# xl-tang3/RCOT

Measured on AMD Instinct MI355X. Metric: 128x128 patches/sec (gen+critic step), higher is better.
Workload: dtype fp32 (exact fp32 MFMA everywhere); 1 GPU; BASELINE configs[1]: Restormer T_net(decoder=True)+F_net(128), denoise_50, RMSprop, paired, B=8/GPU 128x128; global_batch=8, patch=128, parallelism=dp1, gemm_prec=fp32

## Files before the change

### include/rcot_hip.h

```cpp
#ifndef RCOT_HIP_H
#define RCOT_HIP_H
#include <stddef.h>

#ifdef __cplusplus
extern "C" {
#endif

#define RCOT_ABI_VERSION 41

#define RCOT_PREC_FP32 0
#define RCOT_PREC_BF16X3 1
#define RCOT_PREC_BF16X6 2
#define RCOT_PREC_BF16X1 3

int rcot_abi_version(void);
int rcot_debug_nt_coop(int mask);
int rcot_profile_begin(void);
int rcot_profile_end(char* out, int n);
int rcot_last_kernel(char* out, int n);

int rcot_conv1x1_fwd(const float* W, long ldw, const float* X, long sXb, float* Y, long sYb, int B, int Ci, int Co,
                     int N, const float* ln_mu, const float* ln_rs, const float* ln_w, const float* ln_b,
                     const float* R, long sRb, float beta, void* stream);
int rcot_conv1x1_dgrad(const float* W, long ldw, const float* dY, long sdYb, float* dX, long sdXb, int B, int Ci,
                       int Co, int N, float beta, void* stream);
int rcot_conv1x1_wgrad(const float* dY, long sdYb, const float* X, long sXb, float* dW, long ldw, int B, int Ci,
                       int Co, int N, const float* ln_mu, const float* ln_rs, const float* ln_w, const float* ln_b,
                       float beta, float* ws, size_t ws_bytes, int prec, void* stream);
int rcot_conv1x1_wgrad_slabs(const float* dY, long sdYb, const float* X, long sXb, int B, int Ci, int Co, int N,
                             const float* ln_mu, const float* ln_rs, const float* ln_w, const float* ln_b, float* ws,
                             size_t ws_bytes, int prec, int* S, int* ldws, void* stream);
int rcot_conv1x1_dgrad_wgrad_slabs(const float* WP, long ldp, const void* WPs, const float* dY, long sdYb, float* dX, long sdXb,
                                   const float* X, long sXb, int B, int Ci, int Co, int N, const float* ln_mu,
                                   const float* ln_rs, const float* ln_w, const float* ln_b, float* ws, size_t ws_bytes,
                                   float* ws_slabs, size_t ws_slabs_bytes, int prec, int* S, int* ldws, void* stream);

int rcot_bmm_nn(const float* A, long lda, long sAo, long sAi, int transA, const float* Bm, long ldb, long sBo,
                long sBi, float* C, long ldc, long sCo, long sCi, const float* R, long ldr, long sRo, long sRi,
                const float* rowscale, long sSo, long sSi, int Zo, int Zi, int M, int N, int K, float beta,
                void* stream);
int rcot_bmm_nt(const float* A, long lda, long sAo, long sAi, const float* Bm, long ldb, long sBo, long sBi,
                float* C, long ldc, long sCo, long sCi, int Zo, int Zi, int M, int N, int K, float* ws,
                size_t ws_bytes, int prec, void* stream);

int rcot_bmm_nt_slabs(const float* A, long lda, long sAo, long sAi, const float* Bm, long ldb, long sBo, long sBi, int Zo, int Zi,
                      int M, int N, int K, float* ws, size_t ws_bytes, int prec, int* S, int* ldws, void* stream);

int rcot_gemm_kmajor(const float* At, long lda, long sAo, long sAi, int a_rows, const float* Bm, long ldb, long sBo,
                     long sBi, float* C, long ldc, long sCo, long sCi, const float* R, long ldr, long sRo, long sRi,
                     const float* rowscale, long sSo, long sSi, float* ln_mu, float* ln_rs, long sLN, int ln_compute,
                     const float* ln_w, const float* ln_b, const float* AtF, const float* ln_c12, const void* Asplit, int Zo,
                     int Zi, int M, int N, int K, float beta, float* ws, size_t ws_bytes, int prec, void* stream);
typedef struct rcot_kmajor_desc {
    const float* At; long lda, sAo, sAi; int a_rows;
// ... 194 lines not shown
```

### rcot_amd/csrc/pointwise.hip

```cpp
#include <cstdlib>
#include "common.h"
#include "../../include/rcot_hip.h"

using namespace rcot;

namespace {

constexpr int LN_TX = 16, LN_TY = 16, LN_PIX = LN_TX * 4;

__device__ __forceinline__ float4 f4_add(float4 a, float4 b) { return make_float4(a.x + b.x, a.y + b.y, a.z + b.z, a.w + b.w); }

template <int TX>
__device__ __forceinline__ float4 reduce_rows(float4 v, float4* red, int tx, int ty) {
    constexpr int TY = 256 / TX;
    __syncthreads();
    red[ty * TX + tx] = v;
    __syncthreads();
    float4 t = red[tx];
#pragma unroll
    for (int i = 1; i < TY; ++i) t = f4_add(t, red[i * TX + tx]);
    return t;
}

__global__ __launch_bounds__(256) void ln_stats_kernel(const float* __restrict__ x, float* __restrict__ mu,
// ... 159 lines not shown
        if (r < rows) s0 += p[(long)r * C2];
    }
    red[rl][cl] = s0 + s1;
    __syncthreads();
    if (rl == 0 && col < C2) {
        float s = 0.f;
#pragma unroll
        for (int i = 0; i < 32; ++i) s += red[i][cl];
        if (col < C) dw[col] += s;
        else db[col - C] += s;
    }
}

struct SlabSets {
    const float* ws[4];
    float* dst[4];
    int S[4], M[4], N[4], ldws[4];
    int per[4];
    long ldd[4];
    int chunk0[5];
    int n;
};

__global__ __launch_bounds__(1024) void block_param_reduce_kernel(const float* __restrict__ part1, const float* __restrict__ part2,
                                                                  int rows, int C, float* __restrict__ gw1, float* __restrict__ gb1,
                                                                  float* __restrict__ gw2, float* __restrict__ gb2,
                                                                  const float* __restrict__ dWo_part, float* __restrict__ gWo,
                                                                  const float* __restrict__ dtemp_part, float* __restrict__ gtemp,
                                                                  int B, int heads, int nw, SlabSets ss) {
    __shared__ float red[32][33];
    const int nl = (2 * C + 31) / 32;
    const int blk = blockIdx.x;
    if (blk >= 2 * nl + nw) {
        const int cb = blk - 2 * nl - nw;
        int d = 0;
        while (d + 1 < ss.n && cb >= ss.chunk0[d + 1]) ++d;
        const int c = cb - ss.chunk0[d];
        const long mn = (long)ss.M[d] * ss.N[d];
        const long slab = (long)ss.M[d] * ss.ldws[d];
        if (ss.S[d] <= 8) {
            const unsigned Nn = (unsigned)ss.N[d], mnu = (unsigned)mn, S = (unsigned)ss.S[d];
            const unsigned ldw = (unsigned)ss.ldws[d];
            const float* wsb = ss.ws[d];
            float* dstb = ss.dst[d];
            float v[4][8], old[4];
            long doff[4];
            bool ok[4];
#pragma unroll
            for (int j = 0; j < 4; ++j) {
                const unsigned idx = (unsigned)c * 4096u + 1024u * j + threadIdx.x;
                ok[j] = idx < mnu;
                const unsigned ic = ok[j] ? idx : mnu - 1;
                const unsigned m = ic / Nn, n = ic - m * Nn;
                const float* w = wsb + (size_t)m * ldw + n;
                doff[j] = (long)m * ss.ldd[d] + n;
#pragma unroll
                for (unsigned u = 0; u < 8; ++u) {
                    const unsigned uc = u < S ? u : S - 1;
                    v[j][u] = w[(long)uc * slab];
                }
                old[j] = dstb[doff[j]];
            }
#pragma unroll
            for (int j = 0; j < 4; ++j) {
#pragma unroll
                for (unsigned u = 0; u < 8; ++u) v[j][u] = u < S ? v[j][u] : 0.f;
                const float sum = ((v[j][0] + v[j][1]) + (v[j][2] + v[j][3])) + ((v[j][4] + v[j][5]) + (v[j][6] + v[j][7]));
                if (ok[j]) dstb[doff[j]] = old[j] + sum;
            }
            return;
        }
        if (ss.per[d] == 256) {
            const int o = threadIdx.x & 255, q = threadIdx.x >> 8;
            const long idx = (long)c * 256 + o;
            float* part = &red[0][0];
            float a = 0.f;
            int m = 0, n = 0;
            if (idx < mn) {
                m = (int)(idx / ss.N[d]);
                n = (int)(idx - (long)m * ss.N[d]);
                const float* w = ss.ws[d] + (long)m * ss.ldws[d] + n;
                float acc8[8];
#pragma unroll
                for (int u = 0; u < 8; ++u) acc8[u] = 0.f;
                int s = q;
                for (; s + 28 < ss.S[d]; s += 32) {
#pragma unroll
                    for (int u = 0; u < 8; ++u) acc8[u] += w[(long)(s + 4 * u) * slab];
                }
                for (; s < ss.S[d]; s += 4) acc8[0] += w[(long)s * slab];
                a = ((acc8[0] + acc8[1]) + (acc8[2] + acc8[3])) + ((acc8[4] + acc8[5]) + (acc8[6] + acc8[7]));
            }
            part[q * 256 + o] = a;
            __syncthreads();
            if (q == 0 && idx < mn)
                ss.dst[d][(long)m * ss.ldd[d] + n] += (part[o] + part[256 + o]) + (part[512 + o] + part[768 + o]);
            return;
        }
        const int o = threadIdx.x & 255, q = threadIdx.x >> 8;
        const unsigned Nn = (unsigned)ss.N[d], mnu = (unsigned)mn, ldw = (unsigned)ss.ldws[d];
        const int S = ss.S[d];
        float a[4];
        long doff[4];
        bool ok[4];
        const float* w[4];
#pragma unroll
        for (int j = 0; j < 4; ++j) {
            const unsigned idx = (unsigned)c * 1024u + 256u * j + o;
            ok[j] = idx < mnu;
            const unsigned ic = ok[j] ? idx : mnu - 1;
            const unsigned m = ic / Nn, n = ic - m * Nn;
            w[j] = ss.ws[d] + (size_t)m * ldw + n;
            doff[j] = (long)m * ss.ldd[d] + n;
        }
        float acc8[4][8];
#pragma unroll
        for (int j = 0; j < 4; ++j)
#pragma unroll
            for (int u = 0; u < 8; ++u) acc8[j][u] = 0.f;
        int sl = q;
        for (; sl + 28 < S; sl += 32) {
#pragma unroll
            for (int j = 0; j < 4; ++j)
#pragma unroll
                for (int u = 0; u < 8; ++u) acc8[j][u] += w[j][(long)(sl + 4 * u) * slab];
        }
        for (; sl < S; sl += 4) {
#pragma unroll
            for (int j = 0; j < 4; ++j) acc8[j][0] += w[j][(long)sl * slab];
        }
#pragma unroll
        for (int j = 0; j < 4; ++j)
            a[j] = ((acc8[j][0] + acc8[j][1]) + (acc8[j][2] + acc8[j][3])) + ((acc8[j][4] + acc8[j][5]) + (acc8[j][6] + acc8[j][7]));
        __shared__ float part4[4][1024];
#pragma unroll
        for (int j = 0; j < 4; ++j) part4[q][256 * j + o] = a[j];
        __syncthreads();
        {
            const int t = threadIdx.x;
            const unsigned idx = (unsigned)c * 1024u + t;
            if (idx < mnu) {
                const unsigned m = idx / Nn, n = idx - m * Nn;
                ss.dst[d][(long)m * ss.ldd[d] + n] += (part4[0][t] + part4[1][t]) + (part4[2][t] + part4[3][t]);
            }
        }
        (void)doff; (void)ok;
        return;
    }
    if (blk < 2 * nl) {
        const float* part = blk < nl ? part1 : part2;
        float* dw = blk < nl ? gw1 : gw2;
        float* db = blk < nl ? gb1 : gb2;
        const int cb = blk < nl ? blk : blk - nl;
        const int cl = threadIdx.x & 31, rl = threadIdx.x >> 5;
        const int col = cb * 32 + cl, C2 = 2 * C;
        float a8[8];
#pragma unroll
        for (int u = 0; u < 8; ++u) a8[u] = 0.f;
        if (col < C2) {
            const float* p = part + col;
            int r = rl;
            for (; r + 224 < rows; r += 256) {
#pragma unroll
                for (int u = 0; u < 8; ++u) a8[u] += p[(long)(r + 32 * u) * C2];
            }
            for (; r < rows; r += 32) a8[0] += p[(long)r * C2];
        }
        red[rl][cl] = ((a8[0] + a8[1]) + (a8[2] + a8[3])) + ((a8[4] + a8[5]) + (a8[6] + a8[7]));
        __syncthreads();
// ... 5 lines not shown
            else db[col - C] += s;
        }
        return;
    }
    const long n = (long)C * C;
    const long i = (long)(blk - 2 * nl) * 1024 + threadIdx.x;
    if (i < n) {
        float s = 0.f;
        int b = 0;
        for (; b + 8 <= B; b += 8) {
            float v[8];
#pragma unroll
            for (int u = 0; u < 8; ++u) v[u] = dWo_part[(long)(b + u) * n + i];
#pragma unroll
            for (int u = 0; u < 8; ++u) s += v[u];
        }
        for (; b < B; ++b) s += dWo_part[(long)b * n + i];
        gWo[i] += s;
    }
    if (blk == 2 * nl && threadIdx.x < heads) {
        float s = 0.f;
        for (int b = 0; b < B; ++b) s += dtemp_part[(long)b * heads + threadIdx.x];
        gtemp[threadIdx.x] += s;
    }
}

__global__ __launch_bounds__(256) void row_sumsq_kernel(const float* __restrict__ x, float* __restrict__ out, int R,
                                                        int N, long sXb) {
    __shared__ float red[4];
    const int r = blockIdx.x, b = blockIdx.y;
    const float* p = x + (long)b * sXb + (long)r * N;
    float s = 0.f;
#pragma unroll 4
    for (int n = threadIdx.x * 4; n < N; n += 1024) {
        const float4 v = *reinterpret_cast<const float4*>(p + n);
        s += v.x * v.x + v.y * v.y + v.z * v.z + v.w * v.w;
    }
    s = block_sum<256>(s, red);
    if (threadIdx.x == 0) out[(long)b * R + r] = s;
}

__global__ void lrelu_bwd_kernel(const float* __restrict__ dy, const float* __restrict__ a, float* __restrict__ dz,
                                 long n, float slope) {
    for (long i = (long)blockIdx.x * blockDim.x + threadIdx.x; i < n; i += (long)gridDim.x * blockDim.x)
        dz[i] = a[i] > 0.f ? dy[i] : dy[i] * slope;
}
// ... 125 lines not shown
        else if (nc == 6) RCOT_LNB(6, 16);
        else RCOT_LNB(0, 16);
    } else {
        if (nc == 3) RCOT_LNB(3, 4);
        else if (nc == 6) RCOT_LNB(6, 4);
        else RCOT_LNB(0, 4);
    }
#undef RCOT_LNB
    RCOT_LAUNCH_CHECK();
    if (dw) {
        RCOT_LAUNCH(ln_param_reduce_kernel, dim3(cdiv(2 * C, 32)), dim3(1024), 0, (hipStream_t)stream, part, gx * B, C, dw, db);
        RCOT_LAUNCH_CHECK();
    }
    return RCOT_OK;
}

int rcot_ln_bwd_rows(int B, int C, int N) {
    (void)C;
    if (B <= 0 || N <= 0) return 0;
    bool wide;
    return ln_bwd_grid(B, N, &wide) * B;
}

int rcot_block_param_reduce(const float* part1, const float* part2, int rows, int C, float* gw1, float* gb1, float* gw2,
                            float* gb2, const float* dWo_part, float* gWo, const float* dtemp_part, float* gtemp, int B,
                            int heads, const long long* slab_sets, int n_sets, void* stream) {
    if (!part1 || !part2 || !gw1 || !gb1 || !gw2 || !gb2 || !dWo_part || !gWo || !dtemp_part || !gtemp || rows <= 0 || C <= 0 ||
        B <= 0 || heads <= 0 || heads > 1024 || n_sets < 0 || n_sets > 4 || (n_sets && !slab_sets))
        return RCOT_EINVAL;
    const int nl = cdiv(2 * C, 32);
    const int nw = cdiv((long)C * C, 1024);
    SlabSets ss{};
    ss.n = n_sets;
    int chunks = 0;
    for (int d = 0; d < n_sets; ++d) {
        const long long* r = slab_sets + 7 * d;
        ss.ws[d] = reinterpret_cast<const float*>(r[0]);
        ss.S[d] = (int)r[1]; ss.M[d] = (int)r[2]; ss.N[d] = (int)r[3]; ss.ldws[d] = (int)r[4];
        ss.dst[d] = reinterpret_cast<float*>(r[5]);
        ss.ldd[d] = r[6];
        if (!ss.ws[d] || !ss.dst[d] || ss.S[d] <= 0 || ss.M[d] <= 0 || ss.N[d] <= 0 || ss.ldws[d] < ss.N[d]) return RCOT_EINVAL;
        ss.chunk0[d] = chunks;
        const long mn_ = (long)ss.M[d] * ss.N[d];
        ss.per[d] = ss.S[d] <= 8 ? 4096 : (mn_ >= 256 * 1024 ? 1024 : 256);
        chunks += cdiv(mn_, ss.per[d]);
    }
    ss.chunk0[n_sets] = chunks;
    RCOT_LAUNCH(block_param_reduce_kernel, dim3(2 * nl + nw + chunks), dim3(1024), 0, (hipStream_t)stream, part1, part2, rows,
                       C, gw1, gb1, gw2, gb2, dWo_part, gWo, dtemp_part, gtemp, B, heads, nw, ss);
    RCOT_LAUNCH_CHECK();
    return RCOT_OK;
}

int rcot_row_sumsq(const float* x, float* out, int B, int R, int N, long sXb, void* stream) {
    if (!x || !out || B <= 0 || R <= 0 || N <= 0 || (N & 3) || (sXb & 3) || !al16(x) || B > 65535) return RCOT_EINVAL;
    RCOT_LAUNCH(row_sumsq_kernel, dim3(R, B), dim3(256), 0, (hipStream_t)stream, x, out, R, N, sXb);
    RCOT_LAUNCH_CHECK();
    return RCOT_OK;
}

int rcot_lrelu_bwd(const float* dy, const float* a, float* dz, long n, float slope, void* stream) {
    if (!dy || !a || !dz || n <= 0) return RCOT_EINVAL;
    RCOT_LAUNCH(lrelu_bwd_kernel, dim3(grid_for(n)), dim3(256), 0, (hipStream_t)stream, dy, a, dz, n, slope);
    RCOT_LAUNCH_CHECK();
    return RCOT_OK;
}

int rcot_bias_grad(const float* dz, float* db, int B, int C, int P, void* stream) {
    if (!dz || !db || B <= 0 || C <= 0 || P <= 0) return RCOT_EINVAL;
    RCOT_LAUNCH(bias_grad_kernel, dim3(C), dim3(256), 0, (hipStream_t)stream, dz, db, B, C, P);
    RCOT_LAUNCH_CHECK();
    return RCOT_OK;
// ... 48 lines not shown
```

### rcot_amd/lib.py

```python
from __future__ import annotations

import ctypes as C
import os

_HERE = os.path.dirname(os.path.abspath(__file__))
ABI_VERSION = 41
PREC_FP32, PREC_BF16X3, PREC_BF16X6, PREC_BF16X1 = 0, 1, 2, 3
SUMSQ_MAX_PARTS, CB_WORDS = 4096, 16
DECIDE_ADAM0, DECIDE_ADAM1, DECIDE_INHERIT = 1, 2, 4
CB_LR, CB_MAX_NORM, CB_NORM, CB_SCALE, CB_STEPS, CB_CLIPPED, CB_SKIPPED, CB_MAX_SEEN, CB_SKIP, CB_T, CB_BC1, CB_BC2 = 0, 1, 2, 3, 4, 5, 6, 7, 8, 9, 11, 13
SB_WORDS, SB_T, SB_LR, SB_EMA_UPDATES, SB_EMA_DECAY, SB_EMA_OMD = 8, 0, 1, 2, 3, 4
LIB_PATH = os.environ.get("RCOT_LIB") or os.path.join(_HERE, "librcot_hip.so")


class RcotLibraryError(RuntimeError):
    pass


class RcotKernelError(RuntimeError):
    pass


_f = C.c_void_p
_l = C.c_long
_i = C.c_int
_fl = C.c_float
_d = C.c_double
_sz = C.c_size_t

# ... 24 lines not shown
    "rcot_gemm_kmajor": [_f, _l, _l, _l, _i, _f, _l, _l, _l, _f, _l, _l, _l, _f, _l, _l, _l, _f, _l, _l,
                         _f, _f, _l, _i, _f, _f, _f, _f, _f, _i, _i, _i, _i, _i, _fl, _f, _sz, _i, _f],
    "rcot_gemm_kmajor_stats": [_f, _l, _l, _l, _i, _f, _l, _l, _l, _f, _l, _l, _l, _f, _l, _l, _l, _f, _f, _l, _i, _i, _i, _i, _i, _f],
    "rcot_kmajor_desc_size": [],
    "rcot_gemm_kmajor_multi": [_f, _i, _i, _i, _f],
    "rcot_pack_weight": [_f, _l, _i, _i, _f, _f, _f, _f, _f, _f, _f, _f, _f, _f, _f, _f, _f],
    "rcot_pack_weights": [_f, _f, _i, _f],
    "rcot_linear_fwd": [_f, _f, _f, _f, _i, _i, _i, _fl, _f, _sz, _f],
    "rcot_linear_dgrad": [_f, _f, _f, _i, _i, _i, _f, _sz, _f],
    "rcot_linear_wgrad": [_f, _f, _f, _i, _i, _i, _fl, _f],
    "rcot_conv2d_fwd": [_f, _f, _f, _f, _i, _i, _i, _i, _i, _i, _i, _i, _i, _fl, _i, _f, _f, _fl, _f, _sz, _f],
    "rcot_conv2d_dgrad": [_f, _f, _f, _i, _i, _i, _i, _i, _i, _i, _i, _i, _fl, _f, _fl, _f, _sz, _f],
    "rcot_conv2d_wgrad": [_f, _f, _f, _i, _i, _i, _i, _i, _i, _i, _i, _i, _fl, _f, _sz, _f],
    "rcot_conv_pcm_prep": [_f, _f, _l, _i, _i, _i, _i, _i, _f],
    "rcot_conv_pcm_wgrad": [_f, _f, _l, _i, _i, _i, _i, _f, _fl, _f, _sz, _i, _f],
    "rcot_conv_pcm_merge": [_f, _l, _f, _i, _i, _i, _i, _f],
    "rcot_conv_pcm_pack": [_f, _f, _f, _i, _i, _f, _f],
    "rcot_conv_pcm": [_f, _i, _i, _f, _l, _i, _f, _i, _f, _fl, _f, _f, _l, _f, _sz, _f],
    "rcot_pixel_shuffle": [_f, _f, _l, _i, _i, _i, _f],
    "rcot_ln_stats": [_f, _f, _f, _i, _i, _i, _f],
    "rcot_ln_bwd": [_f, _f, _f, _f, _f, _f, _f, _f, _f, _i, _i, _i, _f, _l, _f],
    "rcot_ln_bwd_rows": [_i, _i, _i],
    "rcot_block_param_reduce": [_f, _f, _i, _i, _f, _f, _f, _f, _f, _f, _f, _f, _i, _i, _f, _i, _f],
    "rcot_dwconv3x3": [_f, _f, _f, _i, _i, _i, _i, _i, _f],
    "rcot_gdfn_gate_fwd": [_f, _f, _f, _i, _i, _i, _i, _f],
    "rcot_gdfn_gate_bwd": [_f, _f, _f, _f, _f, _i, _i, _i, _i, _f],
    "rcot_gdfn_bwd": [_f, _f, _f, _f, _f, _f, _i, _i, _i, _i, _f],
    "rcot_dwconv3x3_wgrad": [_f, _f, _f, _i, _i, _i, _i, _f],
    "rcot_dwconv3x3_bwd": [_f, _f, _f, _f, _f, _i, _i, _i, _i, _f],
    "rcot_row_sumsq": [_f, _f, _i, _i, _i, _l, _f],
    "rcot_attn_softmax": [_f, _i, _i, _f, _f, _f, _f, _i, _i, _i, _f],
    "rcot_attn_bwd_small": [_f, _f, _f, _f, _f, _f, _f, _f, _f, _f, _i, _i, _i, _f],
    "rcot_attn_core_fwd": [_f, _l, _f, _f, _l, _f, _f, _f, _f, _l, _l, _i, _i, _i, _i, _f, _sz, _f],
    "rcot_attn_core_bwd": [_f, _i, _i] + [_f] * 12 + [_i, _i, _i, _f],
    "rcot_attn_rows_bwd": [_f, _i, _i] + [_f] * 12 + [_i, _i, _i, _i, _f, _sz, _f],
    "rcot_attn_rows_ws_bytes": [_i, _i, _i, _i],
    "rcot_batch_reduce": [_f, _f, _i, _l, _fl, _f],
    "rcot_lrelu_bwd": [_f, _f, _f, _l, _fl, _f],
    "rcot_bias_grad": [_f, _f, _i, _i, _i, _f],
    "rcot_axpby2d": [_f, _l, _f, _l, _f, _l, _l, _l, _fl, _fl, _f],
    "rcot_fill": [_f, _l, _fl, _f],
    "rcot_lerp": [_f, _f, _f, _f, _i, _l, _f],
    "rcot_gp_penalty": [_f, _f, _f, _f, _i, _l, _fl, _f],
    "rcot_ot_reduce": [_f, _f, _f, _f, _i, _l, _f],
    "rcot_fft_plan": [_i, _f, _i],
    "rcot_ot_spectrum": [_f, _f, _f, _f, _f, _f, _sz, _i, _i, _i, _f],
# ... 86 lines not shown
```

### rcot_amd/net_restormer.py

```python
from __future__ import annotations

from collections import OrderedDict
from typing import Callable, Dict, List, Optional

import numpy as np

import torch

from . import params as P


class ParamStore:

    def __init__(self, be, shapes, live_order: List[str], dead: List[str]):
        self.be = be
        self.shapes = list(shapes)
        self.layout = P.make_layout(shapes, live_order, dead)
        self.flat = be.zeros(self.layout.n_total)
        self.grad = be.zeros(self.layout.n_total)
        self.p: Dict[str, torch.Tensor] = {}
        self.g: Dict[str, torch.Tensor] = {}
        for name, shp in self.shapes:
            o = self.layout.offset[name]
            n = int(np.prod(shp))
# ... 76 lines not shown
            if getattr(be, "x6_packs", False):
                st6, sp6 = be.split6_shapes(*W.shape)
                split6 = (be.zeros(*st6), be.zeros(*sp6), be.zeros(*st6) if folded else None)
            return tuple(be.zeros(*s) for s in be.pack_shapes(*W.shape)) + (fold, (be.zeros(*st), be.zeros(*sp), be.zeros(*st) if folded else None), split6)
        self.pk_qkv, self.pk_o, self.pk_in, self.pk_out = mk(self.Wqkv, True), mk(self.Wo), mk(self.Win, True), mk(self.Wout)

    def pack_items(self):
        return [(self.Wqkv, self.pk_qkv[0], self.pk_qkv[1], (self.w1, self.b1) + self.pk_qkv[2], self.pk_qkv[3], self.pk_qkv[4]),
                (self.Wo, self.pk_o[0], self.pk_o[1], None, self.pk_o[3], self.pk_o[4]),
                (self.Win, self.pk_in[0], self.pk_in[1], (self.w2, self.b2) + self.pk_in[2], self.pk_in[3], self.pk_in[4]),
                (self.Wout, self.pk_out[0], self.pk_out[1], None, self.pk_out[3], self.pk_out[4])]

    def repack(self):
        for W, WT, WP, fold, split, split6 in self.pack_items():
            self.be.pack_weight(W, WT, WP, fold, split, split6)

    def _wgrad(self, dY, X, gW, ln, part):
        be = self.be
        d = be.conv1x1_wgrad_slabs(dY, X, gW, ln=ln, region=(part, 3))
        if d is None:
            be.conv1x1_wgrad(dY, X, gW, ln=ln, beta=1.0)
        return d

    def _dgrad_wgrad(self, slabs, W, dY, dX, X, gW, ln, packed, part):
        be = self.be
        pair = getattr(be, "conv1x1_dgrad_wgrad_slabs", None)
        d = pair(W, dY, dX, X, gW, ln=ln, packed=packed, region=(part, 3)) if pair is not None else None
        if d is not None:
            slabs.append(d)
            return
        hold = (dY, X) + ((ln[0], ln[1]) if ln is not None else ())
        be.side_run(lambda: slabs.append(self._wgrad(dY, X, gW, ln, part)), *hold)
        be.conv1x1_dgrad(W, dY, dX, packed=packed)

    def _woT_heads(self, B):
        return self.pk_o[0].view(self.heads, self.c, self.C).unsqueeze(0).expand(B, -1, -1, -1)

    def _wo_heads(self, B):
        return self.Wo.view(self.C, self.heads, self.c).permute(1, 0, 2).unsqueeze(0).expand(B, -1, -1, -1)

    def _head_cols(self, M):
        return M.view(M.shape[0], self.C, self.heads, self.c).permute(0, 2, 1, 3)

    def _qkv_views(self, u):
        B, C3, H, W = u.shape
        N = H * W
        uu = u.view(B, 3, self.heads, self.c, N)
        return uu[:, 0], uu[:, 1], u.view(B, 3, self.C, N)[:, 2].unsqueeze(1)

    def forward(self, x, save: bool, wmask: Optional[int] = None, in_stats=None, want_stats: bool = False):
        assert not (save and wmask is not None)
        be, C, hd, c, hid = self.be, self.C, self.heads, self.c, self.hid
        B, _, H, W = x.shape
        N = H * W
        fast = be.kmajor_worth(C, N, B)
        pstats = wmask is None and getattr(be, "stats_ok", None) is not None and be.stats_ok(C, N, B)
# ... 33 lines not shown
        pp = be.empty(B, 2 * hid, H, W)
        be.conv1x1_fwd(self.Win, y, pp, ln=(mu2, rs2, self.w2, self.b2), packed=self.pk_in, ln_compute=not (fast and pstats))
        if wmask is not None:
            pp[..., wmask:].zero_()
        gg = be.empty(B, hid, H, W)
        be.gdfn_gate_fwd(pp, self.Wdw2, gg)
        out = be.empty(B, C, H, W)
        if want_stats and pstats and fast:
            self.out_stats = (be.empty(B, N), be.empty(B, N))
            be.conv1x1_fwd(self.Wout, gg, out, R=y, packed=self.pk_out, stats=self.out_stats)
        else:
            be.conv1x1_fwd(self.Wout, gg, out, R=y, packed=self.pk_out)
        ctx = (x, mu1, rs1, t, u, sq, Gn, A, y, mu2, rs2, pp, gg) if save else None
        return out, ctx

    def backward(self, ctx, dout):
        be, C, hd, c, hid = self.be, self.C, self.heads, self.c, self.hid
        x, mu1, rs1, t, u, sq, Gn, A, y, mu2, rs2, pp, gg = ctx
        B, _, H, W = x.shape
        N = H * W
        fast = be.kmajor_worth(C, N, B)
        slabs = []
        dg = be.empty(B, hid, H, W)
        self._dgrad_wgrad(slabs, self.Wout, dout, dg, gg, self.gWout, None, self.pk_out, 0)
        dp = be.empty(B, 2 * hid, H, W)
        be.gdfn_bwd(pp, self.Wdw2, dg, dp, self.gWdw2)
        del dg
        gln = be.empty(B, C, H, W)
        self._dgrad_wgrad(slabs, self.Win, dp, gln, y, self.gWin, (mu2, rs2, self.w2, self.b2), self.pk_in, 1)
        del dp
        dy = be.empty(B, C, H, W)
        be.ln_bwd(gln, y, mu2, rs2, self.w2, dout, dy, None, None, slot=0)
        Q, K, V = self._qkv_views(u)
        dy4 = dy.view(B, 1, C, N)
        Mf = be.empty(B, C, C)
        rows = getattr(be, "attn_rows_route", None)
        dM = be.bmm_nt_slabs(dy4, V) if rows is not None and rows(c, hd) and N <= be.attn_rows_slab_maxn else None
        if dM is None:
            dM = be.empty(B, C, C)
            be.bmm_nt(dy4, V, dM.unsqueeze(1))
        du = be.empty(B, 3 * C, H, W)
        dQ, dK, dV = self._qkv_views(du)
        dWo_part, dtemp_part = be.empty(B, C, C), be.empty(B, hd)
        Eq, EqT = be.empty(B, hd, c, c), be.empty(B, hd, c, c)
        Dq, Dk = be.empty(B, C), be.empty(B, C)
        if be.attn_core_bwd(dM, self.Wo, A, Gn, sq, self.temp, Mf, dWo_part, dtemp_part, Eq, EqT, Dq, Dk):
            pass
        else:
            be.bmm_nn(self._wo_heads(B), A, self._head_cols(Mf))
            dA = be.empty(B, hd, c, c)
            dMh = self._head_cols(dM)
            be.bmm_nn(self._wo_heads(B), dMh, dA, transA=True)
# ... 643 lines not shown
```

### rcot_amd/ops.py

```python
from __future__ import annotations

from typing import Optional, Sequence, Tuple

import os
import struct
import sys

import ctypes as C

import torch

from . import lib as _lib

LN = Optional[Tuple[torch.Tensor, torch.Tensor, torch.Tensor, torch.Tensor]]


ctypes_ll = C.c_longlong


def _ptr(t: Optional[torch.Tensor]):
    return None if t is None else t.data_ptr()


def check_patch_rows(rows, P: int, deg_out, clean_out) -> None:
# ... 161 lines not shown
        self.overlap = os.environ.get("RCOT_OVERLAP", "1") != "0"
        self._raw_events = os.environ.get("RCOT_RAW_EVENTS", "1") != "0"
        self.attn_core_maxn = 4096
        self.ln_fused = True
        self.prod_stats = True
        self._ev_ring, self._ev_next = [], -1
        self.x6_packs = self.prec == _lib.PREC_BF16X6
        self._side = torch.cuda.Stream(device=self.device) if self.overlap else None
        self._ws_side = torch.empty_like(self.ws) if self.overlap else None
        self._ws_slabs_gen = [torch.empty_like(self.ws), torch.empty_like(self.ws)]
        self._held = []
        self._pcm_cache = {}
        self._pcm_pinned = {}
        self._pcm_touched = set()
        self.pcm_pinning = False
        self._plan = None
        self._side_pending = False
        self._ln_scratch = [[torch.empty(1024 * 1024, dtype=torch.float32, device=self.device) for _ in range(2)] for _ in range(2)]
        self._ln_rows = 0
        self._gen = 0
        self._gen_event = [None, None]
        self._held_gen = [[], []]
        self._defer_close_env = os.environ.get("RCOT_DEFER_CLOSE")

    @property
    def defer_close(self):
        if self._defer_close_env is not None:
            return self._defer_close_env != "0"
        return self.prec == _lib.PREC_BF16X6

    def side_run(self, fn, *hold):
        if not self.overlap:
            fn()
            return
        self._handover_to_side()
        ws = self.ws
        self.ws = self._ws_side
        try:
            with torch.cuda.stream(self._side):
                fn()
        finally:
            self.ws = ws
        self._held.extend(hold)
        self._side_pending = True

    def side_join(self):
        if self._side_pending:
            self._handover_from_side()
            self._side_pending = False
        self._held.clear()
        for g in (0, 1):
            self._gen_event[g] = None
# ... 639 lines not shown
            ws, nb, dwp, dbp = sc, sc.numel() * 4, None, None
            self._ln_rows = int(self.L.rcot_ln_bwd_rows(B, Cc, N))
        _lib.check(self.L.rcot_ln_bwd(g.data_ptr(), x.data_ptr(), mu.data_ptr(), rs.data_ptr(), w.data_ptr(), _ptr(dres),
                                      dx.data_ptr(), dwp, dbp, B, Cc, N, ws.data_ptr(), nb, self._st()), "rcot_ln_bwd")

    @property
    def _ws_slabs(self):
        return self._ws_slabs_gen[self._gen]

    def _gen_acquire(self):
        gen = self._gen
        if self._gen_event[gen] is not None:
            if self._side is not None and torch.cuda.current_stream() == self._side:
                return
            ev = self._gen_event[gen]
            if isinstance(ev, _Handover):
                dev = self._dev_index
                self._host(lambda: ev.wait(_raw_stream(dev)))
            else:
                self._host(lambda: torch.cuda.current_stream().wait_event(ev))
            self._gen_event[gen] = None
            self._held_gen[gen].clear()

    def block_param_reduce(self, C, gw1, gb1, gw2, gb2, dWo_part, gWo, dtemp_part, gtemp, slabs=(), close_block=False):
        B, heads = dtemp_part.shape
        slabs = [d for d in slabs if d is not None]
        rows = (ctypes_ll * (7 * len(slabs)))(*[v for d in slabs for v in d]) if slabs else None
        g = self._gen
        sc0, sc1, ln_rows = self._ln_scratch[g][0], self._ln_scratch[g][1], self._ln_rows

        def launch():
            _lib.check(self.L.rcot_block_param_reduce(sc0.data_ptr(), sc1.data_ptr(), ln_rows, C,
                                                      gw1.data_ptr(), gb1.data_ptr(), gw2.data_ptr(), gb2.data_ptr(),
                                                      dWo_part.data_ptr(), gWo.data_ptr(), dtemp_part.data_ptr(), gtemp.data_ptr(), B,
                                                      heads, rows, len(slabs), self._st()), "rcot_block_param_reduce")
        if close_block and self.overlap and self.defer_close:
            self._handover_to_side()
            with torch.cuda.stream(self._side):
                launch()
            if self._raw_events:
                ev, side = self._new_handover(), self._side.cuda_stream
                self._host(lambda: ev.record(side))
            else:
                ev = torch.cuda.Event()
                self._host(lambda: ev.record(self._side))
            self._gen_event[g] = ev
# ... 629 lines not shown
```

### rcot_amd/profiling.py

```python
from __future__ import annotations

import ctypes
from collections import defaultdict
from typing import Dict

import torch

GEMM_OPS = ("gemm_kmajor", "gemm_kmajor_stats", "gemm_kmajor_multi", "conv1x1_fwd", "conv1x1_dgrad", "conv1x1_dgrad_wgrad_slabs", "conv1x1_wgrad", "conv1x1_wgrad_slabs", "bmm_nn", "bmm_nt",
            "bmm_nt_slabs", "linear_fwd", "linear_dgrad",
            "linear_wgrad", "conv2d_fwd", "conv2d_dgrad", "conv2d_wgrad")
OTHER_OPS = ("ln_stats", "ln_bwd", "dwconv3x3", "gdfn_gate_fwd", "gdfn_gate_bwd", "gdfn_bwd", "dwconv3x3_wgrad", "dwconv3x3_bwd", "row_sumsq",
             "attn_softmax", "attn_bwd_small", "batch_reduce", "block_param_reduce", "lrelu_bwd", "bias_grad", "axpby", "fill", "lerp", "gp_penalty",
             "pixel_shuffle", "pack_weight", "ot_reduce", "ot_spectrum", "ot_grad", "rmsprop_step", "adam_step",
             "grad_sumsq", "grad_decide", "rmsprop_step_guarded", "adam_step_guarded")


def _numel(t):
    if not isinstance(t, torch.Tensor):
        return 0
    n = 1
    for sz, st in zip(t.shape, t.stride()):
        if st != 0:
            n *= sz
    return n


def _flops(name, a, kw):
    if name == "conv1x1_dgrad_wgrad_slabs":
        return 4.0 * a[0].shape[0] * a[0].shape[1] * a[1].shape[0] * (a[1].numel() // (a[1].shape[0] * a[1].shape[1]))
    if name.startswith("conv1x1"):
        ts = [t for t in a[:3]]
        w = ts[0] if name not in ("conv1x1_wgrad", "conv1x1_wgrad_slabs") else ts[2]
        x = ts[1]
        return 2.0 * w.shape[0] * w.shape[1] * x.shape[0] * (x.numel() // (x.shape[0] * x.shape[1]))
    if name == "gemm_kmajor_multi":
# ... 47 lines not shown
    def _wrap(self, name, fn):
        gemm = name in GEMM_OPS

        def timed(*a, **kw):
            if self._depth:
                return fn(*a, **kw)
            s, e = torch.cuda.Event(enable_timing=True), torch.cuda.Event(enable_timing=True)
            seq0 = self._kname(self._kbuf, 192) if self._kname is not None else 0
            if name == "block_param_reduce" and kw.get("close_block") and not getattr(self.be, "defer_close", False):
                self.be.side_join()
            s.record()
            self._depth += 1
            try:
                r = fn(*a, **kw)
            finally:
                self._depth -= 1
            e.record()
            sym = name
            if self._kname is not None and self._kname(self._kbuf, 192) != seq0:
                sym = self._kbuf.value.decode()
            nbytes = 4.0 * (sum(_numel(t) for t in a) + sum(_numel(t) for t in kw.values()))
            if name == "gemm_kmajor_multi":
                nbytes = 4.0 * sum(_numel(t) for it in a[0] for t in it)
            ln = kw.get("ln")
            if ln is not None:
                nbytes += 4.0 * sum(_numel(t) for t in ln)
            key = name + str(tuple(tuple(t.shape) for t in (a[:4] if name != "gemm_kmajor_multi" else [it[2] for it in a[0]]) if isinstance(t, torch.Tensor)))
            if ln is not None:
                key += "+ln"
            self.records.append((name, s, e, _flops(name, a, kw) if gemm else 0.0, nbytes, key, sym))
            if key not in self._calls:
                self._calls[key] = (fn, a, kw)
            return r
        return timed

    def remove(self):
        for name, fn in self._orig.items():
            setattr(self.be, name, fn)

    def summary(self) -> Dict[str, dict]:
        torch.cuda.synchronize()
        out = defaultdict(lambda: dict(calls=0, ms=0.0, flops=0.0, bytes=0.0))
        for name, s, e, fl, by, _key, _sym in self.records:
            d = out[name]
            d["calls"] += 1
            d["ms"] += s.elapsed_time(e)
            d["flops"] += fl
            d["bytes"] += by
        return dict(out)

    def by_shape(self, top: int = 25):
        torch.cuda.synchronize()
# ... 55 lines not shown
```

Before: 106.4 patches/s.

## Reduce GDFN weight-grad slabs early on the side stream

Adds a standalone slab-sum reduction kernel, using a persistent grid of up to 64 workgroups, and factors the slab-chunk summation out of block_param_reduce into a shared device function. In the GDFN backward pass, when both wgrad slab sets were produced on the side stream, they are now reduced into the weight gradients right after the second wgrad. This moves the work off the critical path instead of leaving it for the end-of-block param reduce. It is enabled by default for fp32 and bf16x6 and trades an extra kernel launch for overlap with main-stream dgrad work.

Result: faster. 108.3 patches/s (median of 6 runs) (+1.8%).

```diff
diff --git a/include/rcot_hip.h b/include/rcot_hip.h
--- a/include/rcot_hip.h
+++ b/include/rcot_hip.h
@@ -6,7 +6,7 @@
 extern "C" {
 #endif
 
-#define RCOT_ABI_VERSION 41
+#define RCOT_ABI_VERSION 42
 
 #define RCOT_PREC_FP32 0
 #define RCOT_PREC_BF16X3 1
@@ -30,6 +30,7 @@
 int rcot_conv1x1_wgrad_slabs(const float* dY, long sdYb, const float* X, long sXb, int B, int Ci, int Co, int N,
                              const float* ln_mu, const float* ln_rs, const float* ln_w, const float* ln_b, float* ws,
                              size_t ws_bytes, int prec, int* S, int* ldws, void* stream);
+int rcot_slab_sets_reduce(const long long* slab_sets, int n_sets, void* stream);
 int rcot_conv1x1_dgrad_wgrad_slabs(const float* WP, long ldp, const void* WPs, const float* dY, long sdYb, float* dX, long sdXb,
                                    const float* X, long sXb, int B, int Ci, int Co, int N, const float* ln_mu,
                                    const float* ln_rs, const float* ln_w, const float* ln_b, float* ws, size_t ws_bytes,
diff --git a/rcot_amd/csrc/pointwise.hip b/rcot_amd/csrc/pointwise.hip
--- a/rcot_amd/csrc/pointwise.hip
+++ b/rcot_amd/csrc/pointwise.hip
@@ -205,6 +205,122 @@
     int n;
 };
 
+__device__ __forceinline__ void slab_chunk_sum(const SlabSets& ss, int cb) {
+    __shared__ float part4[4][1024];
+    int d = 0;
+    while (d + 1 < ss.n && cb >= ss.chunk0[d + 1]) ++d;
+    const int c = cb - ss.chunk0[d];
+    const long mn = (long)ss.M[d] * ss.N[d];
+    const long slab = (long)ss.M[d] * ss.ldws[d];
+    if (ss.S[d] <= 8) {
+        const unsigned Nn = (unsigned)ss.N[d], mnu = (unsigned)mn, S = (unsigned)ss.S[d];
+        const unsigned ldw = (unsigned)ss.ldws[d];
+        const float* wsb = ss.ws[d];
+        float* dstb = ss.dst[d];
+        float v[4][8], old[4];
+        long doff[4];
+        bool ok[4];
+#pragma unroll
+        for (int j = 0; j < 4; ++j) {
+            const unsigned idx = (unsigned)c * 4096u + 1024u * j + threadIdx.x;
+            ok[j] = idx < mnu;
+            const unsigned ic = ok[j] ? idx : mnu - 1;
+            const unsigned m = ic / Nn, n = ic - m * Nn;
+            const float* w = wsb + (size_t)m * ldw + n;
+            doff[j] = (long)m * ss.ldd[d] + n;
+#pragma unroll
+            for (unsigned u = 0; u < 8; ++u) {
+                const unsigned uc = u < S ? u : S - 1;
+                v[j][u] = w[(long)uc * slab];
+            }
+            old[j] = dstb[doff[j]];
+        }
+#pragma unroll
+        for (int j = 0; j < 4; ++j) {
+#pragma unroll
+            for (unsigned u = 0; u < 8; ++u) v[j][u] = u < S ? v[j][u] : 0.f;
+            const float sum = ((v[j][0] + v[j][1]) + (v[j][2] + v[j][3])) + ((v[j][4] + v[j][5]) + (v[j][6] + v[j][7]));
+            if (ok[j]) dstb[doff[j]] = old[j] + sum;
+        }
+        return;
+    }
+    if (ss.per[d] == 256) {
+        const int o = threadIdx.x & 255, q = threadIdx.x >> 8;
+        const long idx = (long)c * 256 + o;
+        float* part = &part4[0][0];
+        float a = 0.f;
+        int m = 0, n = 0;
+        if (idx < mn) {
+            m = (int)(idx / ss.N[d]);
+            n = (int)(idx - (long)m * ss.N[d]);
+            const float* w = ss.ws[d] + (long)m * ss.ldws[d] + n;
+            float acc8[8];
+#pragma unroll
+            for (int u = 0; u < 8; ++u) acc8[u] = 0.f;
+            int s = q;
+            for (; s + 28 < ss.S[d]; s += 32) {
+#pragma unroll
+                for (int u = 0; u < 8; ++u) acc8[u] += w[(long)(s + 4 * u) * slab];
+            }
+            for (; s < ss.S[d]; s += 4) acc8[0] += w[(long)s * slab];
+            a = ((acc8[0] + acc8[1]) + (acc8[2] + acc8[3])) + ((acc8[4] + acc8[5]) + (acc8[6] + acc8[7]));
+        }
+        part[q * 256 + o] = a;
+        __syncthreads();
+        if (q == 0 && idx < mn)
+            ss.dst[d][(long)m * ss.ldd[d] + n] += (part[o] + part[256 + o]) + (part[512 + o] + part[768 + o]);
+        return;
+    }
+    const int o = threadIdx.x & 255, q = threadIdx.x >> 8;
+    const unsigned Nn = (unsigned)ss.N[d], mnu = (unsigned)mn, ldw = (unsigned)ss.ldws[d];
+    const int S = ss.S[d];
+    float a[4];
+    long doff[4];
+    bool ok[4];
+    const float* w[4];
+#pragma unroll
+    for (int j = 0; j < 4; ++j) {
+        const unsigned idx = (unsigned)c * 1024u + 256u * j + o;
+        ok[j] = idx < mnu;
+        const unsigned ic = ok[j] ? idx : mnu - 1;
+        const unsigned m = ic / Nn, n = ic - m * Nn;
+        w[j] = ss.ws[d] + (size_t)m * ldw + n;
+        doff[j] = (long)m * ss.ldd[d] + n;
+    }
+    float acc8[4][8];
+#pragma unroll
+    for (int j = 0; j < 4; ++j)
+#pragma unroll
+        for (int u = 0; u < 8; ++u) acc8[j][u] = 0.f;
+    int sl = q;
+    for (; sl + 28 < S; sl += 32) {
+#pragma unroll
+        for (int j = 0; j < 4; ++j)
+#pragma unroll
+            for (int u = 0; u < 8; ++u) acc8[j][u] += w[j][(long)(sl + 4 * u) * slab];
+    }
+    for (; sl < S; sl += 4) {
+#pragma unroll
+        for (int j = 0; j < 4; ++j) acc8[j][0] += w[j][(long)sl * slab];
+    }
+#pragma unroll
+    for (int j = 0; j < 4; ++j)
+        a[j] = ((acc8[j][0] + acc8[j][1]) + (acc8[j][2] + acc8[j][3])) + ((acc8[j][4] + acc8[j][5]) + (acc8[j][6] + acc8[j][7]));
+#pragma unroll
+    for (int j = 0; j < 4; ++j) part4[q][256 * j + o] = a[j];
+    __syncthreads();
+    {
+        const int t = threadIdx.x;
+        const unsigned idx = (unsigned)c * 1024u + t;
+        if (idx < mnu) {
+            const unsigned m = idx / Nn, n = idx - m * Nn;
+            ss.dst[d][(long)m * ss.ldd[d] + n] += (part4[0][t] + part4[1][t]) + (part4[2][t] + part4[3][t]);
+        }
+    }
+    (void)doff; (void)ok;
+    return;
+}
+
 __global__ __launch_bounds__(1024) void block_param_reduce_kernel(const float* __restrict__ part1, const float* __restrict__ part2,
                                                                   int rows, int C, float* __restrict__ gw1, float* __restrict__ gb1,
                                                                   float* __restrict__ gw2, float* __restrict__ gb2,
@@ -215,119 +331,7 @@
     const int nl = (2 * C + 31) / 32;
     const int blk = blockIdx.x;
     if (blk >= 2 * nl + nw) {
-        const int cb = blk - 2 * nl - nw;
-        int d = 0;
-        while (d + 1 < ss.n && cb >= ss.chunk0[d + 1]) ++d;
-        const int c = cb - ss.chunk0[d];
-        const long mn = (long)ss.M[d] * ss.N[d];
-        const long slab = (long)ss.M[d] * ss.ldws[d];
-        if (ss.S[d] <= 8) {
-            const unsigned Nn = (unsigned)ss.N[d], mnu = (unsigned)mn, S = (unsigned)ss.S[d];
-            const unsigned ldw = (unsigned)ss.ldws[d];
-            const float* wsb = ss.ws[d];
-            float* dstb = ss.dst[d];
-            float v[4][8], old[4];
-            long doff[4];
-            bool ok[4];
-#pragma unroll
-            for (int j = 0; j < 4; ++j) {
-                const unsigned idx = (unsigned)c * 4096u + 1024u * j + threadIdx.x;
-                ok[j] = idx < mnu;
-                const unsigned ic = ok[j] ? idx : mnu - 1;
-                const unsigned m = ic / Nn, n = ic - m * Nn;
-                const float* w = wsb + (size_t)m * ldw + n;
-                doff[j] = (long)m * ss.ldd[d] + n;
-#pragma unroll
-                for (unsigned u = 0; u < 8; ++u) {
-                    const unsigned uc = u < S ? u : S - 1;
-                    v[j][u] = w[(long)uc * slab];
-                }
-                old[j] = dstb[doff[j]];
-            }
-#pragma unroll
-            for (int j = 0; j < 4; ++j) {
-#pragma unroll
-                for (unsigned u = 0; u < 8; ++u) v[j][u] = u < S ? v[j][u] : 0.f;
-                const float sum = ((v[j][0] + v[j][1]) + (v[j][2] + v[j][3])) + ((v[j][4] + v[j][5]) + (v[j][6] + v[j][7]));
-                if (ok[j]) dstb[doff[j]] = old[j] + sum;
-            }
-            return;
-        }
-        if (ss.per[d] == 256) {
-            const int o = threadIdx.x & 255, q = threadIdx.x >> 8;
-            const long idx = (long)c * 256 + o;
-            float* part = &red[0][0];
-            float a = 0.f;
-            int m = 0, n = 0;
-            if (idx < mn) {
-                m = (int)(idx / ss.N[d]);
-                n = (int)(idx - (long)m * ss.N[d]);
-                const float* w = ss.ws[d] + (long)m * ss.ldws[d] + n;
-                float acc8[8];
-#pragma unroll
-                for (int u = 0; u < 8; ++u) acc8[u] = 0.f;
-                int s = q;
-                for (; s + 28 < ss.S[d]; s += 32) {
-#pragma unroll
-                    for (int u = 0; u < 8; ++u) acc8[u] += w[(long)(s + 4 * u) * slab];
-                }
-                for (; s < ss.S[d]; s += 4) acc8[0] += w[(long)s * slab];
-                a = ((acc8[0] + acc8[1]) + (acc8[2] + acc8[3])) + ((acc8[4] + acc8[5]) + (acc8[6] + acc8[7]));
-            }
-            part[q * 256 + o] = a;
-            __syncthreads();
-            if (q == 0 && idx < mn)
-                ss.dst[d][(long)m * ss.ldd[d] + n] += (part[o] + part[256 + o]) + (part[512 + o] + part[768 + o]);
-            return;
-        }
-        const int o = threadIdx.x & 255, q = threadIdx.x >> 8;
-        const unsigned Nn = (unsigned)ss.N[d], mnu = (unsigned)mn, ldw = (unsigned)ss.ldws[d];
-        const int S = ss.S[d];
-        float a[4];
-        long doff[4];
-        bool ok[4];
-        const float* w[4];
-#pragma unroll
-        for (int j = 0; j < 4; ++j) {
-            const unsigned idx = (unsigned)c * 1024u + 256u * j + o;
-            ok[j] = idx < mnu;
-            const unsigned ic = ok[j] ? idx : mnu - 1;
-            const unsigned m = ic / Nn, n = ic - m * Nn;
-            w[j] = ss.ws[d] + (size_t)m * ldw + n;
-            doff[j] = (long)m * ss.ldd[d] + n;
-        }
-        float acc8[4][8];
-#pragma unroll
-        for (int j = 0; j < 4; ++j)
-#pragma unroll
-            for (int u = 0; u < 8; ++u) acc8[j][u] = 0.f;
-        int sl = q;
-        for (; sl + 28 < S; sl += 32) {
-#pragma unroll
-            for (int j = 0; j < 4; ++j)
-#pragma unroll
-                for (int u = 0; u < 8; ++u) acc8[j][u] += w[j][(long)(sl + 4 * u) * slab];
-        }
-        for (; sl < S; sl += 4) {
-#pragma unroll
-            for (int j = 0; j < 4; ++j) acc8[j][0] += w[j][(long)sl * slab];
-        }
-#pragma unroll
-        for (int j = 0; j < 4; ++j)
-            a[j] = ((acc8[j][0] + acc8[j][1]) + (acc8[j][2] + acc8[j][3])) + ((acc8[j][4] + acc8[j][5]) + (acc8[j][6] + acc8[j][7]));
-        __shared__ float part4[4][1024];
-#pragma unroll
-        for (int j = 0; j < 4; ++j) part4[q][256 * j + o] = a[j];
-        __syncthreads();
-        {
-            const int t = threadIdx.x;
-            const unsigned idx = (unsigned)c * 1024u + t;
-            if (idx < mnu) {
-                const unsigned m = idx / Nn, n = idx - m * Nn;
-                ss.dst[d][(long)m * ss.ldd[d] + n] += (part4[0][t] + part4[1][t]) + (part4[2][t] + part4[3][t]);
-            }
-        }
-        (void)doff; (void)ok;
+        slab_chunk_sum(ss, blk - 2 * nl - nw);
         return;
     }
     if (blk < 2 * nl) {
@@ -379,6 +383,15 @@
         float s = 0.f;
         for (int b = 0; b < B; ++b) s += dtemp_part[(long)b * heads + threadIdx.x];
         gtemp[threadIdx.x] += s;
+    }
+}
+
+constexpr int SLAB_SETS_WGS = 64;
+__global__ __launch_bounds__(1024) void slab_sets_reduce_kernel(SlabSets ss) {
+    const int total = ss.chunk0[ss.n];
+    for (int cb = blockIdx.x; cb < total; cb += gridDim.x) {
+        slab_chunk_sum(ss, cb);
+        __syncthreads();
     }
 }
 
@@ -550,6 +563,25 @@
     return ln_bwd_grid(B, N, &wide) * B;
 }
 
+static int slab_sets_fill(SlabSets& ss, const long long* slab_sets, int n_sets) {
+    ss.n = n_sets;
+    int chunks = 0;
+    for (int d = 0; d < n_sets; ++d) {
+        const long long* r = slab_sets + 7 * d;
+        ss.ws[d] = reinterpret_cast<const float*>(r[0]);
+        ss.S[d] = (int)r[1]; ss.M[d] = (int)r[2]; ss.N[d] = (int)r[3]; ss.ldws[d] = (int)r[4];
+        ss.dst[d] = reinterpret_cast<float*>(r[5]);
+        ss.ldd[d] = r[6];
+        if (!ss.ws[d] || !ss.dst[d] || ss.S[d] <= 0 || ss.M[d] <= 0 || ss.N[d] <= 0 || ss.ldws[d] < ss.N[d]) return -1;
+        ss.chunk0[d] = chunks;
+        const long mn_ = (long)ss.M[d] * ss.N[d];
+        ss.per[d] = ss.S[d] <= 8 ? 4096 : (mn_ >= 256 * 1024 ? 1024 : 256);
+        chunks += cdiv(mn_, ss.per[d]);
+    }
+    ss.chunk0[n_sets] = chunks;
+    return chunks;
+}
+
 int rcot_block_param_reduce(const float* part1, const float* part2, int rows, int C, float* gw1, float* gb1, float* gw2,
                             float* gb2, const float* dWo_part, float* gWo, const float* dtemp_part, float* gtemp, int B,
                             int heads, const long long* slab_sets, int n_sets, void* stream) {
@@ -559,23 +591,20 @@
     const int nl = cdiv(2 * C, 32);
     const int nw = cdiv((long)C * C, 1024);
     SlabSets ss{};
-    ss.n = n_sets;
-    int chunks = 0;
-    for (int d = 0; d < n_sets; ++d) {
-        const long long* r = slab_sets + 7 * d;
-        ss.ws[d] = reinterpret_cast<const float*>(r[0]);
-        ss.S[d] = (int)r[1]; ss.M[d] = (int)r[2]; ss.N[d] = (int)r[3]; ss.ldws[d] = (int)r[4];
-        ss.dst[d] = reinterpret_cast<float*>(r[5]);
-        ss.ldd[d] = r[6];
-        if (!ss.ws[d] || !ss.dst[d] || ss.S[d] <= 0 || ss.M[d] <= 0 || ss.N[d] <= 0 || ss.ldws[d] < ss.N[d]) return RCOT_EINVAL;
-        ss.chunk0[d] = chunks;
-        const long mn_ = (long)ss.M[d] * ss.N[d];
-        ss.per[d] = ss.S[d] <= 8 ? 4096 : (mn_ >= 256 * 1024 ? 1024 : 256);
-        chunks += cdiv(mn_, ss.per[d]);
-    }
-    ss.chunk0[n_sets] = chunks;
+    const int chunks = slab_sets_fill(ss, slab_sets, n_sets);
+    if (chunks < 0) return RCOT_EINVAL;
     RCOT_LAUNCH(block_param_reduce_kernel, dim3(2 * nl + nw + chunks), dim3(1024), 0, (hipStream_t)stream, part1, part2, rows,
                        C, gw1, gb1, gw2, gb2, dWo_part, gWo, dtemp_part, gtemp, B, heads, nw, ss);
+    RCOT_LAUNCH_CHECK();
+    return RCOT_OK;
+}
+
+int rcot_slab_sets_reduce(const long long* slab_sets, int n_sets, void* stream) {
+    if (!slab_sets || n_sets < 1 || n_sets > 4) return RCOT_EINVAL;
+    SlabSets ss{};
+    const int chunks = slab_sets_fill(ss, slab_sets, n_sets);
+    if (chunks < 0) return RCOT_EINVAL;
+    RCOT_LAUNCH(slab_sets_reduce_kernel, dim3(chunks < SLAB_SETS_WGS ? chunks : SLAB_SETS_WGS), dim3(1024), 0, (hipStream_t)stream, ss);
     RCOT_LAUNCH_CHECK();
     return RCOT_OK;
 }
diff --git a/rcot_amd/lib.py b/rcot_amd/lib.py
--- a/rcot_amd/lib.py
+++ b/rcot_amd/lib.py
@@ -4,7 +4,7 @@
 import os
 
 _HERE = os.path.dirname(os.path.abspath(__file__))
-ABI_VERSION = 41
+ABI_VERSION = 42
 PREC_FP32, PREC_BF16X3, PREC_BF16X6, PREC_BF16X1 = 0, 1, 2, 3
 SUMSQ_MAX_PARTS, CB_WORDS = 4096, 16
 DECIDE_ADAM0, DECIDE_ADAM1, DECIDE_INHERIT = 1, 2, 4
@@ -75,6 +75,7 @@
     "rcot_ln_bwd": [_f, _f, _f, _f, _f, _f, _f, _f, _f, _i, _i, _i, _f, _l, _f],
     "rcot_ln_bwd_rows": [_i, _i, _i],
     "rcot_block_param_reduce": [_f, _f, _i, _i, _f, _f, _f, _f, _f, _f, _f, _f, _i, _i, _f, _i, _f],
+    "rcot_slab_sets_reduce": [_f, _i, _f],
     "rcot_dwconv3x3": [_f, _f, _f, _i, _i, _i, _i, _i, _f],
     "rcot_gdfn_gate_fwd": [_f, _f, _f, _i, _i, _i, _i, _f],
     "rcot_gdfn_gate_bwd": [_f, _f, _f, _f, _f, _i, _i, _i, _i, _f],
diff --git a/rcot_amd/net_restormer.py b/rcot_amd/net_restormer.py
--- a/rcot_amd/net_restormer.py
+++ b/rcot_amd/net_restormer.py
@@ -122,16 +122,21 @@
             be.conv1x1_wgrad(dY, X, gW, ln=ln, beta=1.0)
         return d
 
-    def _dgrad_wgrad(self, slabs, W, dY, dX, X, gW, ln, packed, part):
+    def _dgrad_wgrad(self, slabs, W, dY, dX, X, gW, ln, packed, part, then=None):
         be = self.be
         pair = getattr(be, "conv1x1_dgrad_wgrad_slabs", None)
         d = pair(W, dY, dX, X, gW, ln=ln, packed=packed, region=(part, 3)) if pair is not None else None
         if d is not None:
             slabs.append(d)
-            return
+            return False
         hold = (dY, X) + ((ln[0], ln[1]) if ln is not None else ())
-        be.side_run(lambda: slabs.append(self._wgrad(dY, X, gW, ln, part)), *hold)
+        def leaf():
+            slabs.append(self._wgrad(dY, X, gW, ln, part))
+            if then is not None:
+                then()
+        be.side_run(leaf, *hold)
         be.conv1x1_dgrad(W, dY, dX, packed=packed)
+        return True
 
     def _woT_heads(self, B):
         return self.pk_o[0].view(self.heads, self.c, self.C).unsqueeze(0).expand(B, -1, -1, -1)
@@ -211,12 +216,19 @@
         fast = be.kmajor_worth(C, N, B)
         slabs = []
         dg = be.empty(B, hid, H, W)
-        self._dgrad_wgrad(slabs, self.Wout, dout, dg, gg, self.gWout, None, self.pk_out, 0)
+        on_side = self._dgrad_wgrad(slabs, self.Wout, dout, dg, gg, self.gWout, None, self.pk_out, 0)
+        early = getattr(be, "slab_sets_reduce", None) if getattr(be, "early_slab_sums", False) and on_side else None
+
+        def early_sum():
+            if len(slabs) == 2 and slabs[0] is not None and slabs[1] is not None:
+                early(slabs)
+                del slabs[:]
         dp = be.empty(B, 2 * hid, H, W)
         be.gdfn_bwd(pp, self.Wdw2, dg, dp, self.gWdw2)
         del dg
         gln = be.empty(B, C, H, W)
-        self._dgrad_wgrad(slabs, self.Win, dp, gln, y, self.gWin, (mu2, rs2, self.w2, self.b2), self.pk_in, 1)
+        self._dgrad_wgrad(slabs, self.Win, dp, gln, y, self.gWin, (mu2, rs2, self.w2, self.b2), self.pk_in, 1,
+                          then=early_sum if early is not None else None)
         del dp
         dy = be.empty(B, C, H, W)
         be.ln_bwd(gln, y, mu2, rs2, self.w2, dout, dy, None, None, slot=0)
diff --git a/rcot_amd/ops.py b/rcot_amd/ops.py
--- a/rcot_amd/ops.py
+++ b/rcot_amd/ops.py
@@ -207,12 +207,19 @@
         self._gen_event = [None, None]
         self._held_gen = [[], []]
         self._defer_close_env = os.environ.get("RCOT_DEFER_CLOSE")
+        self._early_slabs_env = os.environ.get("RCOT_EARLY_SLABS")
 
     @property
     def defer_close(self):
         if self._defer_close_env is not None:
             return self._defer_close_env != "0"
         return self.prec == _lib.PREC_BF16X6
+
+    @property
+    def early_slab_sums(self):
+        if self._early_slabs_env is not None:
+            return self._early_slabs_env != "0"
+        return self.prec in (_lib.PREC_FP32, _lib.PREC_BF16X6)
 
     def side_run(self, fn, *hold):
         if not self.overlap:
@@ -898,6 +905,13 @@
             self._gen_event[gen] = None
             self._held_gen[gen].clear()
 
+    def slab_sets_reduce(self, slabs):
+        slabs = [d for d in slabs if d is not None]
+        if not slabs:
+            return
+        rows = (ctypes_ll * (7 * len(slabs)))(*[v for d in slabs for v in d])
+        _lib.check(self.L.rcot_slab_sets_reduce(rows, len(slabs), self._st()), "rcot_slab_sets_reduce")
+
     def block_param_reduce(self, C, gw1, gb1, gw2, gb2, dWo_part, gWo, dtemp_part, gtemp, slabs=(), close_block=False):
         B, heads = dtemp_part.shape
         slabs = [d for d in slabs if d is not None]
diff --git a/rcot_amd/profiling.py b/rcot_amd/profiling.py
--- a/rcot_amd/profiling.py
+++ b/rcot_amd/profiling.py
@@ -10,7 +10,7 @@
             "bmm_nt_slabs", "linear_fwd", "linear_dgrad",
             "linear_wgrad", "conv2d_fwd", "conv2d_dgrad", "conv2d_wgrad")
 OTHER_OPS = ("ln_stats", "ln_bwd", "dwconv3x3", "gdfn_gate_fwd", "gdfn_gate_bwd", "gdfn_bwd", "dwconv3x3_wgrad", "dwconv3x3_bwd", "row_sumsq",
-             "attn_softmax", "attn_bwd_small", "batch_reduce", "block_param_reduce", "lrelu_bwd", "bias_grad", "axpby", "fill", "lerp", "gp_penalty",
+             "attn_softmax", "attn_bwd_small", "batch_reduce", "block_param_reduce", "slab_sets_reduce", "lrelu_bwd", "bias_grad", "axpby", "fill", "lerp", "gp_penalty",
              "pixel_shuffle", "pack_weight", "ot_reduce", "ot_spectrum", "ot_grad", "rmsprop_step", "adam_step",
              "grad_sumsq", "grad_decide", "rmsprop_step_guarded", "adam_step_guarded")
 
@@ -104,12 +104,16 @@
             nbytes = 4.0 * (sum(_numel(t) for t in a) + sum(_numel(t) for t in kw.values()))
             if name == "gemm_kmajor_multi":
                 nbytes = 4.0 * sum(_numel(t) for it in a[0] for t in it)
+            if name == "slab_sets_reduce":
+                nbytes = 4.0 * sum(d[1] * d[2] * d[3] + 2 * d[2] * d[3] for d in a[0] if d is not None)
             ln = kw.get("ln")
             if ln is not None:
                 nbytes += 4.0 * sum(_numel(t) for t in ln)
             key = name + str(tuple(tuple(t.shape) for t in (a[:4] if name != "gemm_kmajor_multi" else [it[2] for it in a[0]]) if isinstance(t, torch.Tensor)))
             if ln is not None:
                 key += "+ln"
+            if name == "slab_sets_reduce":
+                key += str(tuple(d[1:4] for d in a[0] if d is not None))
             self.records.append((name, s, e, _flops(name, a, kw) if gemm else 0.0, nbytes, key, sym))
             if key not in self._calls:
                 self._calls[key] = (fn, a, kw)
```
